# hukenovs/blackman_harris_win

Hardware: AMD Instinct MI355X
Metric: window Gsamples/s (BH-7, N=2^26, 32-bit) + fraction of HBM-write roofline (higher is better)
Workload: dtype int64

## Files before the change

### blackman_harris_win_amd/csrc/bhw_build.hip

```cpp
#include "bhw_device.h"

namespace {

template <typename T>
__global__ __launch_bounds__(kBlock) void k_table_build(BhwCordicCfg cfg, uint32_t entries, void *__restrict__ table)
{
    __shared__ T lut_s[32];
    stage_lut<T>(cfg, lut_s);
    const uint32_t u = blockIdx.x * kBlock + threadIdx.x;
    if (u >= entries) return;
    T x, y;
    cordic_q1<T>(lut_s, (T)cfg.x0, (T)((T)u << cfg.z_shl), (int)cfg.n_iter, x, y);
    const int32_t c = (int32_t)(x >> cfg.out_shr), sn = (int32_t)(y >> cfg.out_shr);
    const int2 head = make_int2(__builtin_amdgcn_readfirstlane(c), __builtin_amdgcn_readfirstlane(sn));
    const int4 rec = cfg.tab_dlog > kPackLog ? reinterpret_cast<const int4 *>(cfg.tab_coarse)[u >> fmt_cell_log(cfg.tab_dlog)] : make_int4(0, 0, 0, 0);
    tab_store(table, u, cfg.phi_width - 2 - cfg.z_shr, cfg.tab_split, cfg.tab_dlog, const_cast<void *>(cfg.tab_coarse), c, sn, head, rec,
              cfg.tab_check);
}


template <int NITER, int FMT>
__global__ __launch_bounds__(kBuildThreads) void k_table_build_shared(BhwBuildPlan plan, void *__restrict__ table)
{
    __shared__ int64_t gx[kGroupsPerWg];
    __shared__ int64_t gy[kGroupsPerWg];
    __shared__ int32_t gz[kGroupsPerWg];
    __shared__ int32_t gk[kGroupsPerWg];
    __shared__ uint32_t lut_s[32];
    if (threadIdx.x < 32) lut_s[threadIdx.x] = plan.lut[threadIdx.x];
    __syncthreads();

    constexpr int n_iter = NITER;
    const uint32_t s = plan.z_shl;
    const uint32_t gpw = plan.groups_per_wg;
    const uint32_t group0 = blockIdx.x * gpw;
    const uint32_t n_groups = plan.entries >> 6;

    if (threadIdx.x < gpw) {
        const uint32_t g = group0 + threadIdx.x;
        const uint32_t u_first = g << 6;
        int64_t x = plan.x0, y = plan.x0;
        int32_t zf = (int32_t)((u_first << s) - lut_s[0]);
        const uint32_t span = 63u << s;
        int k = 1;
        bool live = g < n_groups;
        constexpr int kmax = n_iter < kPrefixMax ? n_iter : kPrefixMax;
#pragma unroll
        for (int kk = 1; kk < kmax; ++kk) {
            if (live) {
                const int32_t zl = (int32_t)((uint32_t)zf + span);
                if ((zf < 0) != (zl < 0)) {
                    live = false;
                } else {
                    rot_step(x, y, zf, kk, plan.lut[kk]);
                    k = kk + 1;
                }
            }
        }
        gx[threadIdx.x] = x;
        gy[threadIdx.x] = y;
        gz[threadIdx.x] = zf;
        gk[threadIdx.x] = k;
    }
    __syncthreads();

    const uint32_t wave = __builtin_amdgcn_readfirstlane(threadIdx.x >> 6), lane = threadIdx.x & 63u;
    uint32_t idx_a = lane, idx_m = 64u;
    if (plan.tab_split) {
        const uint32_t e = 1u << plan.log2_entries;
        if (lane & 1u)      { idx_a = (e >> 1) + (lane >> 1); idx_m = 32u; }
        else if (lane & 2u) { idx_a = (e >> 2) + (lane >> 2); idx_m = 16u; }
        else                { idx_a = lane >> 2;              idx_m = 16u; }
    }
    for (uint32_t gi = wave; gi < gpw; gi += kBuildThreads / 64) {
        const uint32_t g = __builtin_amdgcn_readfirstlane(group0 + gi);
        if (g >= n_groups) break;
        int64_t x = gx[gi], y = gy[gi];
        int32_t z = (int32_t)((uint32_t)gz[gi] + (lane << s));
        const int k0 = __builtin_amdgcn_readfirstlane(gk[gi]);
#pragma unroll
        for (int k = 1; k < NITER; ++k) {
            if (k >= kPrefixMax || k >= k0) rot_step(x, y, z, k, plan.lut[k]);
        }
        const int32_t c = (int32_t)(x >> plan.out_shr), sn = (int32_t)(y >> plan.out_shr);
        const int2 head = make_int2(__builtin_amdgcn_readfirstlane(c), __builtin_amdgcn_readfirstlane(sn));
        const uint32_t idx = idx_a + g * idx_m;
        if constexpr (FMT == 4) {
            const uint32_t u = (g << 6) + lane, nmask = 4u * plan.entries - 1u;
            int32_t *d_sin = reinterpret_cast<int32_t *>(table), *d_cos = reinterpret_cast<int32_t *>(const_cast<void *>(plan.tab_coarse));
#pragma unroll
            for (uint32_t q = 0; q < 4u; ++q) {
                int32_t oc, os;
                quadrant_map(q, c, sn, plan.pad0, oc, os);
                const uint32_t i = (q * plan.entries + u - plan.pad) & nmask;
                if (d_sin) d_sin[i] = os;
                if (d_cos) d_cos[i] = oc;
            }
        } else if constexpr (FMT == 0) {
            reinterpret_cast<int2 *>(table)[idx] = make_int2(c, sn);
        } else {
            static_assert(FMT == 1, "k_table_build_shared builds plain and delta16 tables (and the sin / cos sweep) only");
            const int32_t dc = c - head.x, ds = sn - head.y;
            if (plan.check_flag && !(fits_bits(dc, 16) && fits_bits(ds, 16))) atomicOr(plan.check_flag, 1u);
            reinterpret_cast<uint32_t *>(table)[idx] = ((uint32_t)dc & 0xFFFFu) | ((uint32_t)ds << 16);
            if (lane == 0u) reinterpret_cast<int2 *>(const_cast<void *>(plan.tab_coarse))[g] = head;
        }
    }
}

constexpr int kMirrorTail = 6;
constexpr int mirror_gpw(int threads) { return threads / 4; }
constexpr int mirror_heads_max(int threads) { return mirror_gpw(threads) / 2 + 8; }
constexpr int mirror_heads_pad(int threads) { return (mirror_heads_max(threads) + 63) / 64 * 64; }
constexpr int kTailZ = 256;

constexpr int kTailRows = 65;
struct TailD { int8_t v[kTailRows * 64 + 16]; };
constexpr TailD make_tail_d()
{
    TailD t{};
    for (int p = 0; p < 64; ++p)
        for (int v = 0; v < kTailRows; ++v) {
            int d = 0;
            for (int j = 0; j < kMirrorTail; ++j) d += ((p >> j) & 1) ? -(v >> j) : (v >> j);
            t.v[v * 64 + p] = (int8_t)d;
        }
    return t;
}
__device__ const TailD kTailD = make_tail_d();

template <int K, bool ZERO>
__device__ __forceinline__ void rot_narrow(uint32_t &x, uint32_t &y, int32_t &z, uint32_t &zacc, uint32_t lutk)
{
    uint32_t a, b;
    if constexpr (ZERO) {
        asm volatile("v_lshrrev_b32 %[a], %[k], %[y]\n\t"
                     "v_lshrrev_b32 %[b], %[k], %[x]\n\t"
                     "v_min_u32 %[za], %[za], %[z]\n\t"
                     "v_cmpx_gt_i32 vcc, 0, %[z]\n\t"
                     "v_add_u32 %[x], %[x], %[a]\n\t"
                     "v_sub_u32 %[y], %[y], %[b]\n\t"
                     "v_add_u32 %[z], %[z], %[l]\n\t"
                     "s_not_b64 exec, exec\n\t"
                     "v_sub_u32 %[x], %[x], %[a]\n\t"
                     "v_add_u32 %[y], %[y], %[b]\n\t"
                     "v_sub_u32 %[z], %[z], %[l]\n\t"
                     "s_mov_b64 exec, -1"
                     : [x] "+v"(x), [y] "+v"(y), [z] "+v"(z), [za] "+v"(zacc), [a] "=&v"(a), [b] "=&v"(b)
                     : [l] "s"(lutk), [k] "n"(K)
                     : "vcc", "scc");
    } else {
        asm volatile("v_lshrrev_b32 %[a], %[k], %[y]\n\t"
                     "v_lshrrev_b32 %[b], %[k], %[x]\n\t"
                     "v_cmpx_gt_i32 vcc, 0, %[z]\n\t"
                     "v_add_u32 %[x], %[x], %[a]\n\t"
                     "v_sub_u32 %[y], %[y], %[b]\n\t"
                     "v_add_u32 %[z], %[z], %[l]\n\t"
                     "s_not_b64 exec, exec\n\t"
                     "v_sub_u32 %[x], %[x], %[a]\n\t"
                     "v_add_u32 %[y], %[y], %[b]\n\t"
                     "v_sub_u32 %[z], %[z], %[l]\n\t"
                     "s_mov_b64 exec, -1"
                     : [x] "+v"(x), [y] "+v"(y), [z] "+v"(z), [a] "=&v"(a), [b] "=&v"(b)
                     : [l] "s"(lutk), [k] "n"(K)
                     : "vcc", "scc");
    }
}

template <int KA, int NITER>
__device__ __forceinline__ void rot_narrow_block(uint32_t &x, uint32_t &y, int32_t &z, uint32_t &zacc, const uint32_t *lut, int e, uint32_t hi)
{
    uint32_t a, b;
#define BHW_ROT_I(lbl, i, HI_ADD)                                                                                       \
    #lbl ":\n\t"                                                                                                        \
    "v_lshrrev_b32 %[a], %[k" #i "], %[y]\n\t"                                                                          \
    "v_lshrrev_b32 %[b], %[k" #i "], %[x]\n\t"                                                                          \
    HI_ADD                                                                                                             \
    "v_min_u32 %[za], %[za], %[z]\n\t"                                                                                  \
    "v_cmpx_gt_i32 vcc, 0, %[z]\n\t"                                                                                    \
    "v_add_u32 %[x], %[x], %[a]\n\t"                                                                                    \
    "v_sub_u32 %[y], %[y], %[b]\n\t"                                                                                    \
    "v_add_u32 %[z], %[z], %[l" #i "]\n\t"                                                                              \
    "s_not_b64 exec, exec\n\t"                                                                                          \
    "v_sub_u32 %[x], %[x], %[a]\n\t"                                                                                    \
    "v_add_u32 %[y], %[y], %[b]\n\t"                                                                                    \
    "v_sub_u32 %[z], %[z], %[l" #i "]\n\t"                                                                              \
    "s_mov_b64 exec, -1\n"
#define BHW_ROT_PLAIN(i) BHW_ROT_I(i, i, "")
#define BHW_ROT_HI(i) BHW_ROT_I(2##i, i, "v_add_u32 %[b], %[c" #i "], %[b]\n\t")
#define BHW_ROT_DISPATCH(P)                                                                                            \
                 "s_cmp_lt_i32 %[e], 1\n\ts_cbranch_scc1 " #P "0f\n\t"                                                 \
                 "s_cmp_eq_u32 %[e], 1\n\ts_cbranch_scc1 " #P "1f\n\t"                                                 \
                 "s_cmp_eq_u32 %[e], 2\n\ts_cbranch_scc1 " #P "2f\n\t"                                                 \
                 "s_cmp_eq_u32 %[e], 3\n\ts_cbranch_scc1 " #P "3f\n\t"                                                 \
                 "s_cmp_eq_u32 %[e], 4\n\ts_cbranch_scc1 " #P "4f\n\t"                                                 \
                 "s_cmp_eq_u32 %[e], 5\n\ts_cbranch_scc1 " #P "5f\n\t"                                                 \
                 "s_cmp_eq_u32 %[e], 6\n\ts_cbranch_scc1 " #P "6f\n\t"                                                 \
                 "s_cmp_eq_u32 %[e], 7\n\ts_cbranch_scc1 " #P "7f\n\t"                                                 \
                 "s_cmp_eq_u32 %[e], 8\n\ts_cbranch_scc1 " #P "8f\n\t"                                                 \
                 "s_cmp_eq_u32 %[e], 9\n\ts_cbranch_scc1 " #P "9f\n\t"
    constexpr int S = NITER - 1 - KA;
    static_assert(S >= 9 && S <= 30, "bias shifts");
    asm volatile("s_cmp_lg_u32 %[hi], 0\n\ts_cbranch_scc1 100f\n\t"
                 BHW_ROT_DISPATCH()
                 "s_branch 10f\n"
                 BHW_ROT_PLAIN(0) BHW_ROT_PLAIN(1) BHW_ROT_PLAIN(2) BHW_ROT_PLAIN(3) BHW_ROT_PLAIN(4) BHW_ROT_PLAIN(5) BHW_ROT_PLAIN(6) BHW_ROT_PLAIN(7)
                 BHW_ROT_PLAIN(8) BHW_ROT_PLAIN(9)
                 "10:\n\ts_branch 200f\n"
                 "100:\n\t"
                 BHW_ROT_DISPATCH(2)
                 "s_branch 200f\n"
                 BHW_ROT_HI(0) BHW_ROT_HI(1) BHW_ROT_HI(2) BHW_ROT_HI(3) BHW_ROT_HI(4) BHW_ROT_HI(5) BHW_ROT_HI(6) BHW_ROT_HI(7) BHW_ROT_HI(8) BHW_ROT_HI(9)
                 "200:"
                 : [x] "+v"(x), [y] "+v"(y), [z] "+v"(z), [za] "+v"(zacc), [a] "=&v"(a), [b] "=&v"(b)
                 : [e] "s"(e), [hi] "s"(hi), [l0] "s"(lut[KA]), [l1] "s"(lut[KA + 1]), [l2] "s"(lut[KA + 2]), [l3] "s"(lut[KA + 3]), [l4] "s"(lut[KA + 4]),
                   [l5] "s"(lut[KA + 5]), [l6] "s"(lut[KA + 6]), [l7] "s"(lut[KA + 7]), [l8] "s"(lut[KA + 8]), [l9] "s"(lut[KA + 9]),
                   [k0] "n"(KA), [k1] "n"(KA + 1), [k2] "n"(KA + 2), [k3] "n"(KA + 3), [k4] "n"(KA + 4), [k5] "n"(KA + 5), [k6] "n"(KA + 6),
                   [k7] "n"(KA + 7), [k8] "n"(KA + 8), [k9] "n"(KA + 9),
                   [c0] "n"(1 << S), [c1] "n"(1 << (S - 1)), [c2] "n"(1 << (S - 2)), [c3] "n"(1 << (S - 3)), [c4] "n"(1 << (S - 4)),
                   [c5] "n"(1 << (S - 5)), [c6] "n"(1 << (S - 6)), [c7] "n"(1 << (S - 7)), [c8] "n"(1 << (S - 8)), [c9] "n"(1 << (S - 9))
                 : "vcc", "scc");
#undef BHW_ROT_I
#undef BHW_ROT_PLAIN
#undef BHW_ROT_HI
#undef BHW_ROT_DISPATCH
}

#ifdef BHW_BUILD_STAMPS
__device__ unsigned long long *g_build_stamps = nullptr;
#define BHW_STAMP(i) do { if (g_build_stamps && (threadIdx.x & 63u) == 0u) atomicMax(&g_build_stamps[blockIdx.x * 16u + (i)], (unsigned long long)wall_clock64()); } while (0)
#define BHW_STAMP_MIN(i) do { if (g_build_stamps && threadIdx.x == 0u) g_build_stamps[blockIdx.x * 16u + (i)] = (unsigned long long)wall_clock64(); } while (0)
#else
#define BHW_STAMP(i) do { } while (0)
#define BHW_STAMP_MIN(i) do { } while (0)
#endif

template <int BYTES>
__device__ __forceinline__ void table_store(void *__restrict__ table, uint32_t idx, uint32_t v)
{
    if constexpr (BYTES == 1) asm volatile("global_store_byte %0, %1, %2 sc1" :: "v"(idx), "v"(v), "s"(table) : "memory");
    else asm volatile("global_store_short %0, %1, %2 sc1" :: "v"(idx << 1), "v"(v), "s"(table) : "memory");
}

template <int NITER, int FMT, int THREADS>
__global__ __launch_bounds__(THREADS) __attribute__((amdgpu_waves_per_eu(8, 8))) void k_table_build_mirror(BhwBuildPlan plan, void *__restrict__ table)
{
    BHW_STAMP_MIN(0);
#ifdef BHW_BUILD_STAMPS
    if (g_build_stamps && threadIdx.x == 0u) {
        uint32_t hw, xcc;
        asm volatile("s_getreg_b32 %0, hwreg(HW_REG_HW_ID)\n\ts_getreg_b32 %1, hwreg(HW_REG_XCC_ID)" : "=s"(hw), "=s"(xcc));
        g_build_stamps[blockIdx.x * 16u + 6u] = hw;
        g_build_stamps[blockIdx.x * 16u + 7u] = xcc;
    }
#endif
    static_assert(FMT == 2 || FMT == 3 || FMT == 5, "residual / nibble entries");
    static_assert(NITER >= 21 && NITER <= 32, "narrow state: 32-bit words");
    static_assert(THREADS == 256 || THREADS == 1024, "workgroup shapes");
    constexpr uint32_t gpw = mirror_gpw(THREADS);
    constexpr uint32_t kHeads = mirror_heads_max(THREADS), kHeadsPad = mirror_heads_pad(THREADS);
    static_assert(gpw + 2 * kHeadsPad + 64 <= THREADS, "prefix lanes, two ranges of head chains, the tail-table wave");
    __shared__ int64_t gx[gpw];
    __shared__ int64_t gy[gpw];
    __shared__ int32_t gz[gpw];
    __shared__ int32_t gk[gpw];
    __shared__ uint32_t gflag[gpw];
    __shared__ uint32_t lut_s[32];
    __shared__ uint8_t tail_p[2 * kTailZ];
    __shared__ __attribute__((aligned(16))) int8_t tail_d[kTailRows * 64 + 16];
    constexpr uint32_t kWorkMax = 8 * gpw;
    __shared__ uint32_t work_n;
    __shared__ uint32_t work_u[kWorkMax];
    __shared__ uint32_t esc_n;
    __shared__ int4 esc_list[FMT == 5 ? kEscFill : 1];
    __shared__ int4 esc_tab[FMT == 5 ? kEscSlots : 1];
    if (threadIdx.x < 32) lut_s[threadIdx.x] = plan.lut[threadIdx.x];
    if constexpr (FMT == 5) {
        if (threadIdx.x >= 64u && threadIdx.x < 64u + kEscSlots) esc_tab[threadIdx.x - 64u] = make_int4(-1, 0, 0, 0);
    }
#ifdef BHW_BUILD_STAMPS
    if (g_build_stamps && threadIdx.x == 0u) { asm volatile("s_waitcnt lgkmcnt(0)" ::: "memory"); g_build_stamps[blockIdx.x * 16u + 8u] = (unsigned long long)wall_clock64() | (plan.entries & 0u); }
#endif
    constexpr int n_iter = NITER;
    constexpr int KS = NITER - kMirrorTail;
    const uint32_t s = plan.z_shl;
    const uint32_t group0 = blockIdx.x * gpw;
    const uint32_t E = plan.entries;
    const uint32_t n_groups = E >> 7;
    const uint32_t u_lo = group0 << 6;
    const uint32_t u_hi = ((group0 + gpw) << 6) < (n_groups << 6) ? ((group0 + gpw) << 6) : (n_groups << 6);
    const uint32_t m_last = (E >> 1) - 1u;
    if (threadIdx.x == 0) {
        work_n = 0u;
        esc_n = 0u;
        if (u_hi == (E >> 1)) {
            work_u[0] = E >> 1;
            work_n = 1u;
        }
    }
    if (threadIdx.x >= (uint32_t)THREADS - 64u) {
        const uint32_t t3 = threadIdx.x - ((uint32_t)THREADS - 64u);
#pragma unroll
        for (int q = 0; q < 5; ++q)
            if (t3 + 64u * q < (uint32_t)(kTailRows * 64 + 16) / 16u) reinterpret_cast<int4 *>(tail_d)[t3 + 64u * q] = reinterpret_cast<const int4 *>(kTailD.v)[t3 + 64u * q];
#pragma unroll
        for (int q = 0; q < 2 * kTailZ / 64; ++q) {
            const uint32_t zi = t3 + 64u * (uint32_t)q;
            int32_t z = (int32_t)zi - kTailZ;
            uint32_t p = 0u;
#pragma unroll
            for (int j = 0; j < kMirrorTail; ++j) {
                if (z < 0) { p |= 1u << j; z += (int32_t)plan.lut[KS + j]; } else z -= (int32_t)plan.lut[KS + j];
            }
            tail_p[zi] = (uint8_t)p;
        }
        BHW_STAMP(9);
    }


    __shared__ int32_t hc[2][kHeads], hs[2][kHeads];
    const uint32_t d = fmt_cell_log(plan.tab_dlog);
    const uint32_t cells_total = E >> d;
    uint32_t cell_lo[2] = {0u, 0u}, n_cell[2] = {0u, 0u}, r_lo[2] = {u_lo, 0u}, r_hi[2] = {u_hi, 0u};
    {
        const uint32_t a = u_lo > 1u ? u_lo : 1u, b = (u_hi - 1u) < m_last ? (u_hi - 1u) : m_last;
        if (a <= b) { r_lo[1] = E - b; r_hi[1] = E - a + 1u; }
        if (a <= b && b == (E >> 1) - 1u) r_lo[1] = E >> 1;
    }
#pragma unroll
    for (int w = 0; w < 2; ++w)
        if (r_hi[w] > r_lo[w]) {
            cell_lo[w] = r_lo[w] >> d;
            n_cell[w] = ((r_hi[w] - 1u) >> d) - cell_lo[w] + 1u;
        }
    if (threadIdx.x >= gpw && threadIdx.x < gpw + 2u * kHeadsPad) {
        const uint32_t w = (threadIdx.x - gpw) / kHeadsPad;
        const uint32_t t = (threadIdx.x - gpw) % kHeadsPad;
        if (n_cell[w] && t < n_cell[w] + 2u) {
            const int64_t cell = (t <= n_cell[w]) ? (int64_t)cell_lo[w] + t : (int64_t)cell_lo[w] - 1;
            if (cell >= 0 && cell < (int64_t)cells_total) {
                int64_t x = plan.x0, y = plan.x0;
                int32_t z = (int32_t)((((uint32_t)cell << d) << s) - plan.lut[0]);
#pragma unroll
                for (int r = 1; r < n_iter; ++r) rot_step(x, y, z, r, plan.lut[r]);
                hc[w][t] = (int32_t)(x >> plan.out_shr);
                hs[w][t] = (int32_t)(y >> plan.out_shr);
            }
        }
        BHW_STAMP(10);
    }

    constexpr int kcap = KS < kPrefixMax ? KS : kPrefixMax;
    if (threadIdx.x < gpw) {
        const uint32_t g = group0 + threadIdx.x;
        const uint32_t u_first = g << 6;
        int64_t x = plan.x0, y = plan.x0;
        int32_t zf = (int32_t)((u_first << s) - plan.lut[0]);
        const uint32_t span = 63u << s;
        int k = 1;
        bool live = g < n_groups;
        uint32_t zero0 = 0u;
#pragma unroll
        for (int kk = 1; kk < kcap; ++kk) {
            if (live) {
                const int32_t zl = (int32_t)((uint32_t)zf + span);
                if ((zf < 0) != (zl < 0)) {
                    live = false;
                } else {
                    zero0 |= (uint32_t)(zf == 0);
                    rot_step(x, y, zf, kk, plan.lut[kk]);
                    k = kk + 1;
                }
            }
        }
        const int64_t drift = ((int64_t)1 << (NITER - k + 1)) + 2, lim = (int64_t)1 << NITER;
        const bool narrow = x >= drift && y >= drift && x + drift < lim && y + drift < lim;
        constexpr int64_t kBias = (int64_t)1 << (NITER - 1);
        const bool hi = !narrow && k >= KS - 10 && y >= drift && y + drift < lim && x - kBias >= drift && x - kBias + drift < ((int64_t)1 << 32) &&
                        x + drift < lim + ((int64_t)1 << KS);
        gx[threadIdx.x] = hi ? x - kBias : x;
        gy[threadIdx.x] = y;
        gz[threadIdx.x] = zf;
        gk[threadIdx.x] = k;
        gflag[threadIdx.x] = zero0 | (narrow || hi ? 2u : 0u) | (hi ? 4u : 0u);
        BHW_STAMP(11);
    }
    BHW_STAMP(1);
    __syncthreads();

    __shared__ int4 hrec[2][kHeads];
    {
        const uint32_t w = threadIdx.x / kHeadsPad, t = threadIdx.x % kHeadsPad;
        if (w < 2u && t < n_cell[w]) {
            const uint32_t cell = cell_lo[w] + t;
            int4 r;
            if (cell + 1u < cells_total) r = make_int4(hc[w][t], hs[w][t], hc[w][t + 1] - hc[w][t], hs[w][t + 1] - hs[w][t]);
            else {
                const uint32_t tp = t ? t - 1u : n_cell[w] + 1u;
                r = make_int4(hc[w][t], hs[w][t], hc[w][t] - hc[w][tp], hs[w][t] - hs[w][tp]);
            }
            if constexpr (FMT == 5) { r.x += (int32_t)kEscBias; r.y += (int32_t)kEscBias; }
            if constexpr (fmt_is_nibble(FMT)) { r.x -= 8; r.y -= 8; }
            hrec[w][t] = r;
            if constexpr (fmt_is_nibble(FMT)) { r.z *= 2; r.w *= 2; }
            if ((cell << d) >= r_lo[w])
                reinterpret_cast<int4 *>(const_cast<void *>(plan.tab_coarse))[cell] = r;
        }
    }
    __syncthreads();
    BHW_STAMP_MIN(2);
    auto record_of = [&](int w, uint32_t cell) -> int4 { return hrec[w][cell - cell_lo[w]]; };
    auto record = [&](int w, uint32_t cell) -> int4 {
        return record_of(w, __builtin_amdgcn_readfirstlane(cell));
    };

    auto store_entry = [&](uint32_t idx, int32_t c, int32_t sn, const int4 rec, uint32_t pos) {
        if constexpr (FMT == 5) {
            const int2 p = tab_predict(rec, pos, d);
            const uint32_t nc = (uint32_t)(c - p.x), ns = (uint32_t)(sn - p.y);
            uint32_t v = nc | (ns << 4);
            if (__builtin_expect((int)(nc - 1u > 14u) | (int)(ns > 15u), 0)) {
                const uint32_t slot = atomicAdd(&esc_n, 1u);
                if (slot < kEscFill) esc_list[slot] = make_int4((int32_t)idx, c, sn, 0);
                v = kEscMarker;
            }
            table_store<1>(table, idx, v);
        } else if constexpr (FMT == 3) {
            const int2 p = tab_predict(rec, pos, d);
            const uint32_t nc = (uint32_t)(c - p.x), ns = (uint32_t)(sn - p.y);
            if (plan.check_flag && (nc | ns) > 15u) atomicOr(plan.check_flag, 1u);
            table_store<1>(table, idx, nc | (ns << 4));
        } else {
            const int2 p = tab_predict(rec, pos, d);
            const int32_t dc = c - p.x, ds = sn - p.y;
            if (plan.check_flag && !(fits_bits(dc, 8) && fits_bits(ds, 8))) atomicOr(plan.check_flag, 1u);
            table_store<2>(table, idx, ((uint32_t)dc & 0xFFu) | ((uint32_t)ds << 8));
        }
    };

    const uint32_t wave = __builtin_amdgcn_readfirstlane(threadIdx.x >> 6), lane = threadIdx.x & 63u;
    uint32_t idx_a, idx_m, idx_i;
    if (lane & 1u)      { idx_a = (E >> 1) + (lane >> 1); idx_m = 32u; idx_i = E + (E >> 1) - 1u; }
    else if (lane & 2u) { idx_a = (E >> 2) + (lane >> 2); idx_m = 16u; idx_i = (E >> 1) + (E >> 2) - 1u; }
    else                { idx_a = lane >> 2;              idx_m = 16u; idx_i = E >> 2; }
    if (!plan.tab_split) { idx_a = lane; idx_m = 64u; idx_i = E; }
    const uint32_t fmask = (1u << d) - 1u;
    for (uint32_t gi = wave; gi < gpw; gi += THREADS / 64) {
        const uint32_t g = __builtin_amdgcn_readfirstlane(group0 + gi);
        if (g >= n_groups) break;
        {
            const uint32_t it = (gi - wave) / (uint32_t)(THREADS / 64);
            if (it == 0u) __builtin_amdgcn_s_setprio(3);
            else if (it == 4u) __builtin_amdgcn_s_setprio(2);
            else if (it == 8u) __builtin_amdgcn_s_setprio(1);
            else if (it == 12u) __builtin_amdgcn_s_setprio(0);
        }
        const int k0 = __builtin_amdgcn_readfirstlane(gk[gi]);
        const uint32_t gf = __builtin_amdgcn_readfirstlane(gflag[gi]);
        int32_t z = (int32_t)((uint32_t)gz[gi] + (lane << s));
        uint64_t zmask = 0ull;
        int32_t c1, s1, c2, s2;
        bool replay = false;
        if (gf & 2u) {
            uint32_t x = (uint32_t)gx[gi], y = (uint32_t)gy[gi];
            uint32_t zacc = ~0u;
            constexpr int KA = KS - 10;
            static_assert(KA >= 5 && KA < kcap && KS - KA == 10, "ten-rotation block");
            if (k0 < KA) {
#define BHW_NARROW(K) if constexpr (K < KA) { if (K >= k0) rot_narrow<K, true>(x, y, z, zacc, plan.lut[K]); }
                BHW_NARROW(1) BHW_NARROW(2) BHW_NARROW(3) BHW_NARROW(4) BHW_NARROW(5) BHW_NARROW(6) BHW_NARROW(7) BHW_NARROW(8)
                BHW_NARROW(9) BHW_NARROW(10) BHW_NARROW(11) BHW_NARROW(12) BHW_NARROW(13) BHW_NARROW(14) BHW_NARROW(15)
#undef BHW_NARROW
            }
            const bool hi = (gf & 4u) != 0u;
            rot_narrow_block<KA, NITER>(x, y, z, zacc, plan.lut, k0 - KA, hi ? 1u : 0u);
            zmask = __builtin_amdgcn_ballot_w64(zacc == 0u);
            const uint32_t xrow6 = hi ? (1u << (NITER - 1 - KS + 6)) : 0u;
            const uint32_t bias_out = hi ? ((1u << (NITER - 1)) >> plan.out_shr) : 0u;
            static_assert(KS <= 26, "unrolled to rotation 25");
            constexpr uint32_t lowm = (1u << KS) - 1u;
            const uint32_t zi = (uint32_t)(z + kTailZ);
            const uint32_t mx = (x + 128u) & lowm, my = (y + 128u) & lowm;
            const uint32_t unsafe = (uint32_t)((mx < my ? mx : my) < 256u) | (uint32_t)((zi - 1u) >= (uint32_t)(2 * kTailZ - 1));
            if (__builtin_amdgcn_ballot_w64(unsafe != 0u) == 0ull) {
                const uint32_t xx = ((x >> KS) << 6) + xrow6, yy = (y >> KS) << 6;
                const uint32_t p1 = tail_p[zi], p2 = tail_p[2u * kTailZ - zi];
                const int32_t dx1 = tail_d[p1 + yy], dy1 = tail_d[p1 + xx], dx2 = tail_d[p2 + xx], dy2 = tail_d[p2 + yy];
                c1 = (int32_t)(((x - (uint32_t)dx1) >> plan.out_shr) + bias_out);
                s1 = (int32_t)((y + (uint32_t)dy1) >> plan.out_shr);
                c2 = (int32_t)((y - (uint32_t)dx2) >> plan.out_shr);
                s2 = (int32_t)(((x + (uint32_t)dy2) >> plan.out_shr) + bias_out);
            } else if (hi) {
                int64_t xw = (int64_t)x + ((int64_t)1 << (NITER - 1)), yw = (int64_t)y;
                int64_t x2 = yw, y2 = xw;
                int32_t z2 = -z;
#pragma unroll 1
                for (int k = KS; k < NITER; ++k) {
                    rot_step_dyn(xw, yw, z, k, lut_s[k], true);
                    rot_step_dyn(x2, y2, z2, k, lut_s[k], true);
                }
                c1 = (int32_t)(xw >> plan.out_shr); s1 = (int32_t)(yw >> plan.out_shr);
                c2 = (int32_t)(x2 >> plan.out_shr); s2 = (int32_t)(y2 >> plan.out_shr);
            } else {
                uint32_t x2 = y, y2 = x;
                int32_t z2 = -z;
                uint32_t unused = 0u;
#define BHW_NARROW(K) if constexpr (K >= KS && K < NITER) { rot_narrow<K, false>(x, y, z, unused, plan.lut[K]); rot_narrow<K, false>(x2, y2, z2, unused, plan.lut[K]); }
                BHW_NARROW(15) BHW_NARROW(16) BHW_NARROW(17) BHW_NARROW(18) BHW_NARROW(19) BHW_NARROW(20) BHW_NARROW(21) BHW_NARROW(22)
                BHW_NARROW(23) BHW_NARROW(24) BHW_NARROW(25) BHW_NARROW(26) BHW_NARROW(27) BHW_NARROW(28) BHW_NARROW(29) BHW_NARROW(30)
                BHW_NARROW(31)
#undef BHW_NARROW
                c1 = (int32_t)(x >> plan.out_shr); s1 = (int32_t)(y >> plan.out_shr);
                c2 = (int32_t)(x2 >> plan.out_shr); s2 = (int32_t)(y2 >> plan.out_shr);
            }
        } else {
            int64_t x = gx[gi], y = gy[gi];
#pragma unroll 1
            for (int k = k0; k < KS; ++k) {
                zmask |= __builtin_amdgcn_ballot_w64(z == 0);
                rot_step_dyn(x, y, z, k, lut_s[k], k >= kMad24From);
            }
            int64_t x2 = y, y2 = x;
            int32_t z2 = -z;
#pragma unroll 1
            for (int k = KS; k < NITER; ++k) {
                rot_step_dyn(x, y, z, k, lut_s[k], true);
                rot_step_dyn(x2, y2, z2, k, lut_s[k], true);
            }
            c1 = (int32_t)(x >> plan.out_shr); s1 = (int32_t)(y >> plan.out_shr);
            c2 = (int32_t)(x2 >> plan.out_shr); s2 = (int32_t)(y2 >> plan.out_shr);
        }
        const uint32_t g6 = __builtin_amdgcn_readfirstlane(g << 6);
        const uint32_t u = g6 + lane;
        const bool has_image = u >= 1u && u <= m_last;
        bool deferred = false;
        if (zmask != 0ull || gf & 1u) {
            replay = has_image && ((((zmask >> lane) & 1ull) != 0ull) || ((gf & 1u) && lane == 0u));
            if (replay) {
                const uint32_t slot = atomicAdd(&work_n, 1u);
                if (slot < kWorkMax) { work_u[slot] = u; deferred = true; }
                else {
                    int64_t xf = plan.x0, yf = plan.x0;
                    int32_t zf = (int32_t)(((E - u) << s) - lut_s[0]);
#pragma unroll 1
                    for (int r = 1; r < n_iter; ++r) rot_step_dyn(xf, yf, zf, r, lut_s[r], r >= kMad24From);
                    c2 = (int32_t)(xf >> plan.out_shr);
                    s2 = (int32_t)(yf >> plan.out_shr);
                }
            }
        }
        const uint32_t idx = fmt_is_nibble(FMT) ? (g << 6) + lane : idx_a + g * idx_m;
        store_entry(idx, c1, s1, record(0, g6 >> d), (g6 & fmask) + lane);
        if (has_image && !deferred) {
            const uint32_t um = E - u;
            const uint32_t top = E - g6, cell_a = (top - 63u) >> d, cell_b = top >> d;
            const uint32_t cell_c = cell_a >= cell_lo[1] ? cell_a : cell_lo[1];
            int4 rec2 = record(1, cell_c);
            if (__builtin_amdgcn_readfirstlane(cell_b) != __builtin_amdgcn_readfirstlane(cell_c)) {
                const int4 rb = record(1, cell_b);
                if (lane == 0u) rec2 = rb;
            }
            store_entry(fmt_is_nibble(FMT) ? E - idx : idx_i - idx, c2, s2, rec2, um & fmask);
        }
    }
    BHW_STAMP_MIN(3);
    BHW_STAMP(4);
    __syncthreads();
    const uint32_t n_work = work_n < kWorkMax ? work_n : kWorkMax;
    for (uint32_t i = threadIdx.x; i < n_work; i += THREADS) {
        const uint32_t um = E - work_u[i];
        int64_t xf = plan.x0, yf = plan.x0;
        int32_t zf = (int32_t)((um << s) - plan.lut[0]);
#pragma unroll
        for (int r = 1; r < n_iter; ++r) rot_step(xf, yf, zf, r, plan.lut[r]);
        store_entry(tab_index(um, plan.log2_entries, plan.tab_split), (int32_t)(xf >> plan.out_shr), (int32_t)(yf >> plan.out_shr), record_of(1, um >> d), um & fmask);
    }
    if constexpr (FMT == 5) {
        __syncthreads();
        const uint32_t n_esc = esc_n < kEscFill ? esc_n : kEscFill;
        uint32_t tid = threadIdx.x;
        asm volatile("" : "+v"(tid));
        if (tid < n_esc) {
            const int4 it = esc_list[tid];
            uint32_t h = esc_slot((uint32_t)it.x);
#pragma unroll 1
            for (uint32_t i = 0; i < kEscSlots; ++i) {
                const uint32_t was = atomicCAS(reinterpret_cast<uint32_t *>(&esc_tab[h].x), ~0u, (uint32_t)it.x);
                if (was == ~0u || was == (uint32_t)it.x) { esc_tab[h].y = it.y; esc_tab[h].z = it.z; break; }
                h = (h + 1u) & (kEscSlots - 1u);
            }
        }
        __syncthreads();
        if (tid < kEscSlots) reinterpret_cast<int4 *>(plan.tab_esc)[(size_t)blockIdx.x * kEscSlots + tid] = esc_tab[tid];
        if (tid == 0u && esc_n > kEscFill && plan.check_flag) atomicOr(plan.check_flag, 1u);
    }
    BHW_STAMP(5);
}

template <int NITER>
__global__ __launch_bounds__(kBlock) void k_table_build_plain(BhwCordicCfg cfg, uint32_t entries, int2 *__restrict__ table)
{
    __shared__ uint32_t lut_s[32];
    if (threadIdx.x < 32) lut_s[threadIdx.x] = (uint32_t)cfg.lut[threadIdx.x];
    __syncthreads();
    const uint32_t u = blockIdx.x * kBlock + threadIdx.x;
    if (u >= entries) return;
    int64_t x = cfg.x0, y = cfg.x0;
    int32_t z = (int32_t)((u << cfg.z_shl) - lut_s[0]);
#pragma unroll
    for (int r = 1; r < NITER; ++r) rot_step(x, y, z, r, lut_s[r]);
    table[u] = make_int2((int32_t)(x >> cfg.out_shr), (int32_t)(y >> cfg.out_shr));
}

}


int bhwk_sincos_sweep(const BhwLaunch &l, const BhwCordicCfg &c, uint64_t theta0, int32_t *d_sin, int32_t *d_cos)
{
    hipStream_t st = (hipStream_t)l.stream;
    BhwBuildPlan plan;
    for (uint32_t k = 0; k < 32; ++k) plan.lut[k] = (uint32_t)c.lut[k];
    plan.entries = 1u << (c.phi_width - 2);
    plan.n_iter = c.n_iter;
    plan.z_shl = c.z_shl;
    plan.out_shr = c.out_shr;
    plan.log2_entries = c.phi_width - 2;
    plan.tab_split = 0;
    plan.tab_dlog = 0;
    plan.pad0 = c.ones_neg;
    plan.tab_coarse = d_cos;
    plan.x0 = c.x0;
    plan.check_flag = nullptr;
    plan.tab_esc = nullptr;
    const unsigned groups = plan.entries >> 6;
    plan.groups_per_wg = groups >= 64u * 1024u ? 64u : groups >= 16u * 1024u ? 16u : 4u;
    plan.pad = (uint32_t)(theta0 & ((1ull << c.phi_width) - 1ull));
    const dim3 grid((groups + plan.groups_per_wg - 1) / plan.groups_per_wg), block(kBuildThreads);
    if (!with_int_range<7, 32>(c.n_iter, [&](auto N) { launch(k_table_build_shared<N, 4>, grid, block, st, plan, (void *)d_sin); }))
        return (int)hipErrorInvalidValue;
    return finish(hipSuccess);
}

#ifdef BHW_BUILD_STAMPS
extern "C" int bhw_dbg_build_stamps(void *d_words)
{
    unsigned long long *p = (unsigned long long *)d_words;
    return (int)hipMemcpyToSymbol(HIP_SYMBOL(g_build_stamps), &p, sizeof p);
}
#endif

int bhwk_table_build(const BhwLaunch &l, const BhwCordicCfg &c_in, int32_t *d_table)
{
    const BhwCordicCfg c = table_layout(c_in);
    hipStream_t st = (hipStream_t)l.stream;
    const uint32_t entries = 1u << (c.phi_width - 2 - c.z_shr);
    const bool fits = (c.dat_width + c.out_shr <= 34);
    if (fits && c.n_iter >= 7 && entries < (1u << 20) && c.tab_dlog == 0 && !c.tab_split) {
        const dim3 grid(grid_for(entries)), block(kBlock);
        if (!with_int_range<7, 32>(c.n_iter, [&](auto N) { launch(k_table_build_plain<N>, grid, block, st, c, entries, (int2 *)d_table); }))
            return (int)hipErrorInvalidValue;
        return finish(hipSuccess);
    }
    if (entries >= 64 && fits && c.n_iter >= 2) {
        BhwBuildPlan plan;
        for (uint32_t k = 0; k < 32; ++k) plan.lut[k] = (uint32_t)c.lut[k];
        plan.entries = entries;
        plan.n_iter = c.n_iter;
        plan.z_shl = c.z_shl;
        plan.out_shr = c.out_shr;
        plan.log2_entries = c.phi_width - 2 - c.z_shr;
        plan.tab_split = c.tab_split;
        plan.tab_dlog = c.tab_dlog;
        plan.pad0 = 0;
        plan.tab_coarse = c.tab_coarse;
        plan.x0 = c.x0;
        plan.check_flag = c.tab_check;
        plan.tab_esc = const_cast<void *>(c.tab_esc);
        const unsigned groups = entries >> 6;
        plan.groups_per_wg = groups >= 64u * 1024u ? 64u : groups >= 16u * 1024u ? 16u : 4u;
        plan.pad = 0;
        const dim3 grid((groups + plan.groups_per_wg - 1) / plan.groups_per_wg), block(kBuildThreads);
        const int fmt = fmt_of(c.tab_dlog);
        if (c.n_iter < 21 && fmt != 0) return (int)hipErrorInvalidValue;
        if (bhwk_build_mirror_applies(c, entries)) {
            const unsigned own_groups = entries >> 7;
            const unsigned threads = bhwk_build_mirror_threads(entries);
            const unsigned mgpw = (unsigned)mirror_gpw((int)threads);
            const dim3 mgrid((own_groups + mgpw - 1) / mgpw), mblock(threads);
            plan.groups_per_wg = mgpw;
            const bool listed = with_int_range<21, 32>(c.n_iter, [&](auto N) {
                with_int_or_last<2, 3, 5>(fmt, [&](auto F) {
                    with_int_or_last<1024, 256>((int)threads, [&](auto T) {
                        launch(k_table_build_mirror<N, F, T>, mgrid, mblock, st, plan, (void *)d_table);
                    });
                });
            });
            return listed ? finish(hipSuccess) : (int)hipErrorInvalidValue;
        }
        if (fmt > 1) return (int)hipErrorInvalidValue;
        const bool listed = with_int_range<7, 32>(c.n_iter, [&](auto N) {
            if constexpr (N < 21) launch(k_table_build_shared<N, 0>, grid, block, st, plan, (void *)d_table);
            else with_int_or_last<0, 1>(fmt, [&](auto F) { launch(k_table_build_shared<N, F>, grid, block, st, plan, (void *)d_table); });
        });
        return listed ? finish(hipSuccess) : (int)hipErrorInvalidValue;
    }
    if (c.tab_dlog > kPackLog) return (int)hipErrorInvalidValue;
    if (c.wide) launch(k_table_build<int64_t>, dim3(grid_for(entries)), dim3(kBlock), st, c, entries, (void *)d_table);
    else        launch(k_table_build<int32_t>, dim3(grid_for(entries)), dim3(kBlock), st, c, entries, (void *)d_table);
    return finish(hipSuccess);
}
```

Baseline: 704.2.

## Pack mirror-build group state into int4 and strength-reduce per-group indexing

```diff
diff --git a/blackman_harris_win_amd/csrc/bhw_build.hip b/blackman_harris_win_amd/csrc/bhw_build.hip
--- a/blackman_harris_win_amd/csrc/bhw_build.hip
+++ b/blackman_harris_win_amd/csrc/bhw_build.hip
@@ -168,7 +168,7 @@
 }
 
 template <int KA, int NITER>
-__device__ __forceinline__ void rot_narrow_block(uint32_t &x, uint32_t &y, int32_t &z, uint32_t &zacc, const uint32_t *lut, int e, uint32_t hi)
+__device__ __forceinline__ void rot_narrow_block(uint32_t &x, uint32_t &y, int32_t &z, uint32_t &zacc, const uint32_t (&l)[10], int e, uint32_t hi)
 {
     uint32_t a, b;
 #define BHW_ROT_I(lbl, i, HI_ADD)                                                                                       \
@@ -213,8 +213,8 @@
                  BHW_ROT_HI(0) BHW_ROT_HI(1) BHW_ROT_HI(2) BHW_ROT_HI(3) BHW_ROT_HI(4) BHW_ROT_HI(5) BHW_ROT_HI(6) BHW_ROT_HI(7) BHW_ROT_HI(8) BHW_ROT_HI(9)
                  "200:"
                  : [x] "+v"(x), [y] "+v"(y), [z] "+v"(z), [za] "+v"(zacc), [a] "=&v"(a), [b] "=&v"(b)
-                 : [e] "s"(e), [hi] "s"(hi), [l0] "s"(lut[KA]), [l1] "s"(lut[KA + 1]), [l2] "s"(lut[KA + 2]), [l3] "s"(lut[KA + 3]), [l4] "s"(lut[KA + 4]),
-                   [l5] "s"(lut[KA + 5]), [l6] "s"(lut[KA + 6]), [l7] "s"(lut[KA + 7]), [l8] "s"(lut[KA + 8]), [l9] "s"(lut[KA + 9]),
+                 : [e] "s"(e), [hi] "s"(hi), [l0] "s"(l[0]), [l1] "s"(l[1]), [l2] "s"(l[2]), [l3] "s"(l[3]), [l4] "s"(l[4]),
+                   [l5] "s"(l[5]), [l6] "s"(l[6]), [l7] "s"(l[7]), [l8] "s"(l[8]), [l9] "s"(l[9]),
                    [k0] "n"(KA), [k1] "n"(KA + 1), [k2] "n"(KA + 2), [k3] "n"(KA + 3), [k4] "n"(KA + 4), [k5] "n"(KA + 5), [k6] "n"(KA + 6),
                    [k7] "n"(KA + 7), [k8] "n"(KA + 8), [k9] "n"(KA + 9),
                    [c0] "n"(1 << S), [c1] "n"(1 << (S - 1)), [c2] "n"(1 << (S - 2)), [c3] "n"(1 << (S - 3)), [c4] "n"(1 << (S - 4)),
@@ -260,11 +260,8 @@
     constexpr uint32_t gpw = mirror_gpw(THREADS);
     constexpr uint32_t kHeads = mirror_heads_max(THREADS), kHeadsPad = mirror_heads_pad(THREADS);
     static_assert(gpw + 2 * kHeadsPad + 64 <= THREADS, "prefix lanes, two ranges of head chains, the tail-table wave");
-    __shared__ int64_t gx[gpw];
-    __shared__ int64_t gy[gpw];
-    __shared__ int32_t gz[gpw];
-    __shared__ int32_t gk[gpw];
-    __shared__ uint32_t gflag[gpw];
+    __shared__ int4 gst[gpw];
+    __shared__ int2 ghi[gpw];
     __shared__ uint32_t lut_s[32];
     __shared__ uint8_t tail_p[2 * kTailZ];
     __shared__ __attribute__((aligned(16))) int8_t tail_d[kTailRows * 64 + 16];
@@ -378,11 +375,10 @@
         constexpr int64_t kBias = (int64_t)1 << (NITER - 1);
         const bool hi = !narrow && k >= KS - 10 && y >= drift && y + drift < lim && x - kBias >= drift && x - kBias + drift < ((int64_t)1 << 32) &&
                         x + drift < lim + ((int64_t)1 << KS);
-        gx[threadIdx.x] = hi ? x - kBias : x;
-        gy[threadIdx.x] = y;
-        gz[threadIdx.x] = zf;
-        gk[threadIdx.x] = k;
-        gflag[threadIdx.x] = zero0 | (narrow || hi ? 2u : 0u) | (hi ? 4u : 0u);
+        const int64_t xp = hi ? x - kBias : x;
+        const uint32_t flags = zero0 | (narrow || hi ? 2u : 0u) | (hi ? 4u : 0u) | (g == 0u ? 8u : 0u);
+        gst[threadIdx.x] = make_int4((int32_t)xp, (int32_t)y, zf, (int32_t)((uint32_t)k | (flags << 8)));
+        ghi[threadIdx.x] = make_int2((int32_t)(xp >> 32), (int32_t)(y >> 32));
         BHW_STAMP(11);
     }
     BHW_STAMP(1);
@@ -410,11 +406,8 @@
     __syncthreads();
     BHW_STAMP_MIN(2);
     auto record_of = [&](int w, uint32_t cell) -> int4 { return hrec[w][cell - cell_lo[w]]; };
-    auto record = [&](int w, uint32_t cell) -> int4 {
-        return record_of(w, __builtin_amdgcn_readfirstlane(cell));
-    };
-
-    auto store_entry = [&](uint32_t idx, int32_t c, int32_t sn, const int4 rec, uint32_t pos) {
+
+    auto store_entry = [&](auto CHECKED, uint32_t idx, int32_t c, int32_t sn, const int4 rec, uint32_t pos) {
         if constexpr (FMT == 5) {
             const int2 p = tab_predict(rec, pos, d);
             const uint32_t nc = (uint32_t)(c - p.x), ns = (uint32_t)(sn - p.y);
@@ -428,12 +421,16 @@
         } else if constexpr (FMT == 3) {
             const int2 p = tab_predict(rec, pos, d);
             const uint32_t nc = (uint32_t)(c - p.x), ns = (uint32_t)(sn - p.y);
-            if (plan.check_flag && (nc | ns) > 15u) atomicOr(plan.check_flag, 1u);
+            if constexpr (decltype(CHECKED)::value) {
+                if (plan.check_flag && (nc | ns) > 15u) atomicOr(plan.check_flag, 1u);
+            }
             table_store<1>(table, idx, nc | (ns << 4));
         } else {
             const int2 p = tab_predict(rec, pos, d);
             const int32_t dc = c - p.x, ds = sn - p.y;
-            if (plan.check_flag && !(fits_bits(dc, 8) && fits_bits(ds, 8))) atomicOr(plan.check_flag, 1u);
+            if constexpr (decltype(CHECKED)::value) {
+                if (plan.check_flag && !(fits_bits(dc, 8) && fits_bits(ds, 8))) atomicOr(plan.check_flag, 1u);
+            }
             table_store<2>(table, idx, ((uint32_t)dc & 0xFFu) | ((uint32_t)ds << 8));
         }
     };
@@ -445,124 +442,156 @@
     else                { idx_a = lane >> 2;              idx_m = 16u; idx_i = E >> 2; }
     if (!plan.tab_split) { idx_a = lane; idx_m = 64u; idx_i = E; }
     const uint32_t fmask = (1u << d) - 1u;
-    for (uint32_t gi = wave; gi < gpw; gi += THREADS / 64) {
-        const uint32_t g = __builtin_amdgcn_readfirstlane(group0 + gi);
-        if (g >= n_groups) break;
-        {
-            const uint32_t it = (gi - wave) / (uint32_t)(THREADS / 64);
-            if (it == 0u) __builtin_amdgcn_s_setprio(3);
-            else if (it == 4u) __builtin_amdgcn_s_setprio(2);
-            else if (it == 8u) __builtin_amdgcn_s_setprio(1);
-            else if (it == 12u) __builtin_amdgcn_s_setprio(0);
-        }
-        const int k0 = __builtin_amdgcn_readfirstlane(gk[gi]);
-        const uint32_t gf = __builtin_amdgcn_readfirstlane(gflag[gi]);
-        int32_t z = (int32_t)((uint32_t)gz[gi] + (lane << s));
-        uint64_t zmask = 0ull;
-        int32_t c1, s1, c2, s2;
-        bool replay = false;
-        if (gf & 2u) {
-            uint32_t x = (uint32_t)gx[gi], y = (uint32_t)gy[gi];
-            uint32_t zacc = ~0u;
-            constexpr int KA = KS - 10;
-            static_assert(KA >= 5 && KA < kcap && KS - KA == 10, "ten-rotation block");
-            if (k0 < KA) {
-#define BHW_NARROW(K) if constexpr (K < KA) { if (K >= k0) rot_narrow<K, true>(x, y, z, zacc, plan.lut[K]); }
-                BHW_NARROW(1) BHW_NARROW(2) BHW_NARROW(3) BHW_NARROW(4) BHW_NARROW(5) BHW_NARROW(6) BHW_NARROW(7) BHW_NARROW(8)
-                BHW_NARROW(9) BHW_NARROW(10) BHW_NARROW(11) BHW_NARROW(12) BHW_NARROW(13) BHW_NARROW(14) BHW_NARROW(15)
+    constexpr uint32_t kWaves = THREADS / 64;
+    static_assert(gpw == 16u * kWaves, "a wave walks 16 groups: four at each priority");
+    constexpr bool kWholeCells = THREADS % (1 << 9) == 0;
+    const uint32_t gi_end = group0 >= n_groups ? 0u : n_groups - group0 < gpw ? n_groups - group0 : gpw;
+    const uint32_t zlane = lane << s;
+    const uint32_t cell_step = ((uint32_t)THREADS >> d) << 4;
+    constexpr int KA = KS - 10;
+    static_assert(KA >= 5 && KA < kcap && KS - KA == 10, "ten-rotation block");
+    uint32_t rom[10];
+#pragma unroll
+    for (int i = 0; i < 10; ++i) {
+        rom[i] = __builtin_amdgcn_readfirstlane(lut_s[KA + i]);
+        asm volatile("" : "+s"(rom[i]));
+    }
+    auto build_groups = [&](auto CHECKED) {
+        uint32_t u = ((group0 + wave) << 6) + lane;
+        uint32_t st_off = wave * (uint32_t)sizeof(int4);
+        asm volatile("" : "+v"(st_off));
+        uint32_t idx = idx_a + (group0 + wave) * idx_m;
+        uint32_t off1, pos1, off2, pos2;
+        auto cells_of = [&]() {
+            const uint32_t um = E - u;
+            pos1 = u & fmask;
+            off1 = ((u >> d) - cell_lo[0]) << 4;
+            pos2 = um & fmask;
+            off2 = ((um >> d) - cell_lo[1]) << 4;
+        };
+        cells_of();
+        uint32_t gi = wave;
+#pragma unroll 1
+        for (uint32_t quarter = 0; quarter < 4u; ++quarter) {
+            if (quarter == 0u) __builtin_amdgcn_s_setprio(3);
+            else if (quarter == 1u) __builtin_amdgcn_s_setprio(2);
+            else if (quarter == 2u) __builtin_amdgcn_s_setprio(1);
+            else __builtin_amdgcn_s_setprio(0);
+            const uint32_t q_end = (quarter + 1u) * 4u * kWaves < gi_end ? (quarter + 1u) * 4u * kWaves : gi_end;
+#pragma unroll 1
+            for (; gi < q_end; gi += kWaves) {
+                const int4 st = *reinterpret_cast<const int4 *>(reinterpret_cast<const char *>(gst) + st_off);
+                const uint32_t kf = __builtin_amdgcn_readfirstlane((uint32_t)st.w);
+                const int k0 = (int)(kf & 0xFFu);
+                const uint32_t gf = kf >> 8;
+                int32_t z = (int32_t)((uint32_t)st.z + zlane);
+                uint64_t zmask = 0ull;
+                int32_t c1, s1, c2, s2;
+                if (gf & 2u) {
+                    uint32_t x = (uint32_t)st.x, y = (uint32_t)st.y;
+                    uint32_t zacc = ~0u;
+                    if (k0 < KA) {
+#define BHW_NARROW(K) if constexpr (K < KA) { if (K >= k0) rot_narrow<K, true>(x, y, z, zacc, K < 9 ? (uint32_t)__builtin_amdgcn_readfirstlane(lut_s[K]) : plan.lut[K]); }
+                        BHW_NARROW(1) BHW_NARROW(2) BHW_NARROW(3) BHW_NARROW(4) BHW_NARROW(5) BHW_NARROW(6) BHW_NARROW(7) BHW_NARROW(8)
+                        BHW_NARROW(9) BHW_NARROW(10) BHW_NARROW(11) BHW_NARROW(12) BHW_NARROW(13) BHW_NARROW(14) BHW_NARROW(15)
 #undef BHW_NARROW
-            }
-            const bool hi = (gf & 4u) != 0u;
-            rot_narrow_block<KA, NITER>(x, y, z, zacc, plan.lut, k0 - KA, hi ? 1u : 0u);
-            zmask = __builtin_amdgcn_ballot_w64(zacc == 0u);
-            const uint32_t xrow6 = hi ? (1u << (NITER - 1 - KS + 6)) : 0u;
-            const uint32_t bias_out = hi ? ((1u << (NITER - 1)) >> plan.out_shr) : 0u;
-            static_assert(KS <= 26, "unrolled to rotation 25");
-            constexpr uint32_t lowm = (1u << KS) - 1u;
-            const uint32_t zi = (uint32_t)(z + kTailZ);
-            const uint32_t mx = (x + 128u) & lowm, my = (y + 128u) & lowm;
-            const uint32_t unsafe = (uint32_t)((mx < my ? mx : my) < 256u) | (uint32_t)((zi - 1u) >= (uint32_t)(2 * kTailZ - 1));
-            if (__builtin_amdgcn_ballot_w64(unsafe != 0u) == 0ull) {
-                const uint32_t xx = ((x >> KS) << 6) + xrow6, yy = (y >> KS) << 6;
-                const uint32_t p1 = tail_p[zi], p2 = tail_p[2u * kTailZ - zi];
-                const int32_t dx1 = tail_d[p1 + yy], dy1 = tail_d[p1 + xx], dx2 = tail_d[p2 + xx], dy2 = tail_d[p2 + yy];
-                c1 = (int32_t)(((x - (uint32_t)dx1) >> plan.out_shr) + bias_out);
-                s1 = (int32_t)((y + (uint32_t)dy1) >> plan.out_shr);
-                c2 = (int32_t)((y - (uint32_t)dx2) >> plan.out_shr);
-                s2 = (int32_t)(((x + (uint32_t)dy2) >> plan.out_shr) + bias_out);
-            } else if (hi) {
-                int64_t xw = (int64_t)x + ((int64_t)1 << (NITER - 1)), yw = (int64_t)y;
-                int64_t x2 = yw, y2 = xw;
-                int32_t z2 = -z;
+                    }
+                    const uint32_t hi = (gf >> 2) & 1u;
+                    rot_narrow_block<KA, NITER>(x, y, z, zacc, rom, k0 - KA, hi);
+                    zmask = __builtin_amdgcn_ballot_w64(zacc == 0u);
+                    const uint32_t xrow6 = hi << (NITER - 1 - KS + 6);
+                    const uint32_t bias_out = (hi << (NITER - 1)) >> plan.out_shr;
+                    static_assert(KS <= 26, "unrolled to rotation 25");
+                    constexpr uint32_t lowm = (1u << KS) - 1u;
+                    const uint32_t zi = (uint32_t)(z + kTailZ);
+                    const uint32_t mx = (x + 128u) & lowm, my = (y + 128u) & lowm;
+                    const uint32_t unsafe = (uint32_t)((mx < my ? mx : my) < 256u) | (uint32_t)((zi - 1u) >= (uint32_t)(2 * kTailZ - 1));
+                    if (__builtin_expect(__builtin_amdgcn_ballot_w64(unsafe != 0u) == 0ull, 1)) {
+                        const uint32_t xx = ((x >> KS) << 6) + xrow6, yy = (y >> KS) << 6;
+                        const uint32_t p1 = tail_p[zi], p2 = tail_p[2u * kTailZ - zi];
+                        const int32_t dx1 = tail_d[p1 + yy], dy1 = tail_d[p1 + xx], dx2 = tail_d[p2 + xx], dy2 = tail_d[p2 + yy];
+                        c1 = (int32_t)(((x - (uint32_t)dx1) >> plan.out_shr) + bias_out);
+                        s1 = (int32_t)((y + (uint32_t)dy1) >> plan.out_shr);
+                        c2 = (int32_t)((y - (uint32_t)dx2) >> plan.out_shr);
+                        s2 = (int32_t)(((x + (uint32_t)dy2) >> plan.out_shr) + bias_out);
+                    } else if (hi) {
+                        int64_t xw = (int64_t)x + ((int64_t)1 << (NITER - 1)), yw = (int64_t)y;
+                        int64_t x2 = yw, y2 = xw;
+                        int32_t z2 = -z;
 #pragma unroll 1
-                for (int k = KS; k < NITER; ++k) {
-                    rot_step_dyn(xw, yw, z, k, lut_s[k], true);
-                    rot_step_dyn(x2, y2, z2, k, lut_s[k], true);
+                        for (int k = KS; k < NITER; ++k) {
+                            rot_step_dyn(xw, yw, z, k, lut_s[k], true);
+                            rot_step_dyn(x2, y2, z2, k, lut_s[k], true);
+                        }
+                        c1 = (int32_t)(xw >> plan.out_shr); s1 = (int32_t)(yw >> plan.out_shr);
+                        c2 = (int32_t)(x2 >> plan.out_shr); s2 = (int32_t)(y2 >> plan.out_shr);
+                    } else {
+                        uint32_t x2 = y, y2 = x;
+                        int32_t z2 = -z;
+                        uint32_t unused = 0u;
+#define BHW_NARROW(K) if constexpr (K >= KS && K < NITER) { rot_narrow<K, false>(x, y, z, unused, plan.lut[K]); rot_narrow<K, false>(x2, y2, z2, unused, plan.lut[K]); }
+                        BHW_NARROW(15) BHW_NARROW(16) BHW_NARROW(17) BHW_NARROW(18) BHW_NARROW(19) BHW_NARROW(20) BHW_NARROW(21) BHW_NARROW(22)
+                        BHW_NARROW(23) BHW_NARROW(24) BHW_NARROW(25) BHW_NARROW(26) BHW_NARROW(27) BHW_NARROW(28) BHW_NARROW(29) BHW_NARROW(30)
+                        BHW_NARROW(31)
+#undef BHW_NARROW
+                        c1 = (int32_t)(x >> plan.out_shr); s1 = (int32_t)(y >> plan.out_shr);
+                        c2 = (int32_t)(x2 >> plan.out_shr); s2 = (int32_t)(y2 >> plan.out_shr);
+                    }
+                } else {
+                    const int2 high = ghi[gi];
+                    int64_t x = (int64_t)(((uint64_t)(uint32_t)high.x << 32) | (uint32_t)st.x), y = (int64_t)(((uint64_t)(uint32_t)high.y << 32) | (uint32_t)st.y);
+#pragma unroll 1
+                    for (int k = k0; k < KS; ++k) {
+                        zmask |= __builtin_amdgcn_ballot_w64(z == 0);
+                        rot_step_dyn(x, y, z, k, lut_s[k], k >= kMad24From);
+                    }
+                    int64_t x2 = y, y2 = x;
+                    int32_t z2 = -z;
+#pragma unroll 1
+                    for (int k = KS; k < NITER; ++k) {
+                        rot_step_dyn(x, y, z, k, lut_s[k], true);
+                        rot_step_dyn(x2, y2, z2, k, lut_s[k], true);
+                    }
+                    c1 = (int32_t)(x >> plan.out_shr); s1 = (int32_t)(y >> plan.out_shr);
+                    c2 = (int32_t)(x2 >> plan.out_shr); s2 = (int32_t)(y2 >> plan.out_shr);
                 }
-                c1 = (int32_t)(xw >> plan.out_shr); s1 = (int32_t)(yw >> plan.out_shr);
-                c2 = (int32_t)(x2 >> plan.out_shr); s2 = (int32_t)(y2 >> plan.out_shr);
-            } else {
-                uint32_t x2 = y, y2 = x;
-                int32_t z2 = -z;
-                uint32_t unused = 0u;
-#define BHW_NARROW(K) if constexpr (K >= KS && K < NITER) { rot_narrow<K, false>(x, y, z, unused, plan.lut[K]); rot_narrow<K, false>(x2, y2, z2, unused, plan.lut[K]); }
-                BHW_NARROW(15) BHW_NARROW(16) BHW_NARROW(17) BHW_NARROW(18) BHW_NARROW(19) BHW_NARROW(20) BHW_NARROW(21) BHW_NARROW(22)
-                BHW_NARROW(23) BHW_NARROW(24) BHW_NARROW(25) BHW_NARROW(26) BHW_NARROW(27) BHW_NARROW(28) BHW_NARROW(29) BHW_NARROW(30)
-                BHW_NARROW(31)
-#undef BHW_NARROW
-                c1 = (int32_t)(x >> plan.out_shr); s1 = (int32_t)(y >> plan.out_shr);
-                c2 = (int32_t)(x2 >> plan.out_shr); s2 = (int32_t)(y2 >> plan.out_shr);
-            }
-        } else {
-            int64_t x = gx[gi], y = gy[gi];
+                const uint32_t own_idx = fmt_is_nibble(FMT) ? u : idx;
+                store_entry(CHECKED, own_idx, c1, s1, *reinterpret_cast<const int4 *>(reinterpret_cast<const char *>(hrec[0]) + off1), pos1);
+                auto store_image = [&]() {
+                    store_entry(CHECKED, fmt_is_nibble(FMT) ? E - u : idx_i - idx, c2, s2,
+                                *reinterpret_cast<const int4 *>(reinterpret_cast<const char *>(hrec[1]) + off2), pos2);
+                };
+                const uint32_t events = (uint32_t)zmask | (uint32_t)(zmask >> 32) | (gf & 9u);
+                if (events == 0u) {
+                    store_image();
+                } else {
+                    const bool replay = u != 0u && ((((zmask >> lane) & 1ull) != 0ull) || ((gf & 1u) && lane == 0u));
+                    bool deferred = false;
+                    if (replay) {
+                        const uint32_t slot = atomicAdd(&work_n, 1u);
+                        if (slot < kWorkMax) { work_u[slot] = u; deferred = true; }
+                        else {
+                            int64_t xf = plan.x0, yf = plan.x0;
+                            int32_t zf = (int32_t)(((E - u) << s) - lut_s[0]);
 #pragma unroll 1
-            for (int k = k0; k < KS; ++k) {
-                zmask |= __builtin_amdgcn_ballot_w64(z == 0);
-                rot_step_dyn(x, y, z, k, lut_s[k], k >= kMad24From);
-            }
-            int64_t x2 = y, y2 = x;
-            int32_t z2 = -z;
-#pragma unroll 1
-            for (int k = KS; k < NITER; ++k) {
-                rot_step_dyn(x, y, z, k, lut_s[k], true);
-                rot_step_dyn(x2, y2, z2, k, lut_s[k], true);
-            }
-            c1 = (int32_t)(x >> plan.out_shr); s1 = (int32_t)(y >> plan.out_shr);
-            c2 = (int32_t)(x2 >> plan.out_shr); s2 = (int32_t)(y2 >> plan.out_shr);
-        }
-        const uint32_t g6 = __builtin_amdgcn_readfirstlane(g << 6);
-        const uint32_t u = g6 + lane;
-        const bool has_image = u >= 1u && u <= m_last;
-        bool deferred = false;
-        if (zmask != 0ull || gf & 1u) {
-            replay = has_image && ((((zmask >> lane) & 1ull) != 0ull) || ((gf & 1u) && lane == 0u));
-            if (replay) {
-                const uint32_t slot = atomicAdd(&work_n, 1u);
-                if (slot < kWorkMax) { work_u[slot] = u; deferred = true; }
-                else {
-                    int64_t xf = plan.x0, yf = plan.x0;
-                    int32_t zf = (int32_t)(((E - u) << s) - lut_s[0]);
-#pragma unroll 1
-                    for (int r = 1; r < n_iter; ++r) rot_step_dyn(xf, yf, zf, r, lut_s[r], r >= kMad24From);
-                    c2 = (int32_t)(xf >> plan.out_shr);
-                    s2 = (int32_t)(yf >> plan.out_shr);
+                            for (int r = 1; r < n_iter; ++r) rot_step_dyn(xf, yf, zf, r, lut_s[r], r >= kMad24From);
+                            c2 = (int32_t)(xf >> plan.out_shr);
+                            s2 = (int32_t)(yf >> plan.out_shr);
+                        }
+                    }
+                    if (u != 0u && !deferred) store_image();
                 }
-            }
-        }
-        const uint32_t idx = fmt_is_nibble(FMT) ? (g << 6) + lane : idx_a + g * idx_m;
-        store_entry(idx, c1, s1, record(0, g6 >> d), (g6 & fmask) + lane);
-        if (has_image && !deferred) {
-            const uint32_t um = E - u;
-            const uint32_t top = E - g6, cell_a = (top - 63u) >> d, cell_b = top >> d;
-            const uint32_t cell_c = cell_a >= cell_lo[1] ? cell_a : cell_lo[1];
-            int4 rec2 = record(1, cell_c);
-            if (__builtin_amdgcn_readfirstlane(cell_b) != __builtin_amdgcn_readfirstlane(cell_c)) {
-                const int4 rb = record(1, cell_b);
-                if (lane == 0u) rec2 = rb;
-            }
-            store_entry(fmt_is_nibble(FMT) ? E - idx : idx_i - idx, c2, s2, rec2, um & fmask);
-        }
-    }
+                u += (uint32_t)THREADS;
+                st_off += kWaves * (uint32_t)sizeof(int4);
+                idx += kWaves * idx_m;
+                if constexpr (kWholeCells) { off1 += cell_step; off2 -= cell_step; }
+                else cells_of();
+            }
+        }
+    };
+    if constexpr (FMT == 5) build_groups(std::false_type{});
+    else if (plan.check_flag) build_groups(std::true_type{});
+    else build_groups(std::false_type{});
     BHW_STAMP_MIN(3);
     BHW_STAMP(4);
     __syncthreads();
@@ -573,7 +602,7 @@
         int32_t zf = (int32_t)((um << s) - plan.lut[0]);
 #pragma unroll
         for (int r = 1; r < n_iter; ++r) rot_step(xf, yf, zf, r, plan.lut[r]);
-        store_entry(tab_index(um, plan.log2_entries, plan.tab_split), (int32_t)(xf >> plan.out_shr), (int32_t)(yf >> plan.out_shr), record_of(1, um >> d), um & fmask);
+        store_entry(std::true_type{}, tab_index(um, plan.log2_entries, plan.tab_split), (int32_t)(xf >> plan.out_shr), (int32_t)(yf >> plan.out_shr), record_of(1, um >> d), um & fmask);
     }
     if constexpr (FMT == 5) {
         __syncthreads();
```

New measurement: 734.8, median of 6. +4.3%, better.
